# georgeretsi/smirk

Hardware: AMD Instinct MI355X
Metric: faces/sec (encode+FLAME+render+generate) @224x224 (higher is better)
Workload: dtype f32 results; encoder + generator convs as split-fp16 x3 MFMA with f32 accumulate (fp32-class error), FLAME / raster f32; 1 GPU; BASELINE config 4: full inference incl. SmirkGenerator re-synthesis, 1024-frame batch sharded over the GPUs; global_batch=1024, micro_batch=1024, image=224x224, parallelism=dp1, rccl_ranks_seen=1, collective=none (1 GPU), hw_queues=4

## Files before the change

### smirk_amd/csrc/conv_common.h

```cpp
#pragma once
#include "common.h"

#define CV_BK 32

typedef _Float16 half8 __attribute__((ext_vector_type(8)));

struct ConvArgs {
    SmirkConvDesc d;
    const float *in0, *in1, *w, *scale, *shift, *residual;
    float* out;
    int M, N, K, Cin;
    float* stats;
    int psh;
};

__device__ __forceinline__ void row_to_pixel(int m, int HoWo, int Wo, int psh, int& b, int& oy, int& ox) {
    b = m / HoWo;
    const int rem = m - b * HoWo;
    const int t = rem >> (2 * psh), in = rem & ((1 << (2 * psh)) - 1);
    const int tpr = Wo >> psh, ty = t / tpr, tx = t - ty * tpr;
    oy = (ty << psh) + (in >> psh);
    ox = (tx << psh) + (in & ((1 << psh) - 1));
}

// ... 66 lines not shown

static inline void conv_prof_next(const char* name, const ConvArgs& a) {
    if (!g_smirk_prof_on) return;
    const double px = (double)a.d.B * a.d.H * a.d.W;
    smirk_prof_next(name, 2.0 * a.M * a.N * a.K, 4.0 * (px * a.Cin + (double)a.M * a.N + (double)a.N * a.K + (a.residual ? (double)a.M * a.N : 0.0)));
}

bool smirk_conv3x3_ring64_eligible(const SmirkConvDesc* d, bool has_residual);
int smirk_conv3x3_ring64_launch(const SmirkConvDesc* d, const void* in0, const void* in1, const void* w, const float* scale, const float* shift, void* out,
                                void* pooled, hipStream_t st, float* stats = nullptr, int* stats_rows = nullptr);
bool smirk_conv3x3_upcat_eligible(int c, int H, int W);
size_t smirk_conv3x3_upcat_weff_bytes(int c);
size_t smirk_conv3x3_upcat_shift_bytes(int c);
int smirk_conv3x3_upcat_launch(int c, const void* d, const void* e, const SmirkConvLayer* up, const SmirkConvLayer* conv, void* out, int B, int H, int W,
                               void* weff, void* shift4, hipStream_t st);
bool smirk_conv3x3_patch_eligible(const SmirkConvDesc* d, bool has_residual);
int smirk_conv3x3_patch_launch(const SmirkConvDesc* d, const void* in0, const void* in1, const void* w, const float* scale,
                               const float* shift, void* out, hipStream_t st, const float* fw, const float* fb, float* fout,
                               int fcout);
#define HS_BM 256
#define HS_WGM 4
bool smirk_conv_halo_eligible(const ConvArgs& a);
int smirk_conv_halo_launch(const ConvArgs& a, hipStream_t st, bool x1);
bool smirk_conv_pp_eligible(const ConvArgs& a);
int smirk_conv_pp_launch(const ConvArgs& a, hipStream_t st);
```

### smirk_amd/csrc/conv_halo.hip

```cpp
#include <stdio.h>
#include <type_traits>

#include "conv_common.h"

#define HS_BN 128
#define HS_NSTAGE 3
#define HS_BRING_BYTES (HS_NSTAGE * HS_BN * 128)
#define HS_EPI_LD (2 * 32 + 4)
#define HS_DEFAULT_EB 0

typedef __attribute__((address_space(3))) void* hs_lptr_t;

template <int K>
using hs_ic = std::integral_constant<int, K>;

__device__ __forceinline__ int hs_b_off(int row, int stage, int piece) {
    return ((((row >> 3) * HS_NSTAGE + stage) << 8) + ((row & 7) << 5) + ((piece ^ ((row >> 1) & 7)) << 2)) * 4;
}

template <int NPA, int EB, bool X1, bool STATS = false>
__device__ __forceinline__ void conv_halo_body(const ConvArgs& a) {
    constexpr int NL = 3;
    extern __shared__ __attribute__((aligned(16))) float hs_smem[];
    char* lds = (char*)hs_smem;
    constexpr int ABUF = NPA * 8 * 1024;
    constexpr int ASTRIDE = ABUF + 128;
    constexpr int A0 = HS_BRING_BYTES;
    const SmirkConvDesc& d = a.d;
    const int tid = threadIdx.x, lane = tid & 63, wave = tid >> 6;
    const int swave = __builtin_amdgcn_readfirstlane(wave);
    const int wm = wave >> 1, wn = wave & 1;
    const int group = swave >> 2;
    const int ntn = a.N / HS_BN;
    const int logical = xcd_logical(blockIdx.x, gridDim.x);
    const int m0 = (logical / ntn) * HS_BM, n0 = (logical % ntn) * HS_BN;
    const int W = d.W, HW = d.H * d.W;
    const int fr = lane & 31, hb = lane >> 5;

    if (tid < 64) *(float*)(lds + A0 + (tid >> 5) * ASTRIDE + ABUF + (tid & 31) * 4) = 0.f;

    unsigned tabA[9];
    unsigned bB[2];
#pragma unroll
    for (int j = 0; j < 2; ++j) bB[j] = (unsigned)hs_b_off((wn * 2 + j) * 32 + fr, 0, 2 * hb);

    const int pos = lane & 7, lrow = lane >> 3;
    const unsigned colA16 = (unsigned)(pos ^ ((4 * (swave & 1) + (lrow >> 1)) & 7)) * 16u;
    const int qv0 = m0 - (W + 1) + 8 * swave + lrow;
    const int npix = d.B * HW;
    unsigned voffB[2];
#pragma unroll
    for (int p = 0; p < 2; ++p) {
        const int brow = 8 * (swave + 8 * p) + lrow;
        voffB[p] = ((unsigned)min(n0 + brow, a.N - 1) * (unsigned)a.K + (unsigned)(pos ^ ((brow >> 1) & 7)) * 4u) * 4u;
    }
    const __amdgpu_buffer_rsrc_t rs0 = __builtin_amdgcn_make_buffer_rsrc((void*)a.in0, (short)0, (int)((long long)npix * d.C0 * 4), 0x00020000);
    const __amdgpu_buffer_rsrc_t rs1 = __builtin_amdgcn_make_buffer_rsrc((void*)(d.C1 > 0 ? a.in1 : a.in0), (short)0,
                                                                         (int)((long long)npix * (d.C1 > 0 ? d.C1 : d.C0) * 4), 0x00020000);
    const __amdgpu_buffer_rsrc_t rsw = __builtin_amdgcn_make_buffer_rsrc((void*)a.w, (short)0, (int)((long long)a.N * a.K * 4), 0x00020000);
    const int sh0 = 31 - __builtin_clz((unsigned)d.C0) + 2, sh1 = d.C1 > 0 ? 31 - __builtin_clz((unsigned)d.C1) + 2 : sh0;
    const int ncc = (d.C0 + d.C1) / CV_BK;

    auto dmaA = [&](int cc, int abase, auto kc) {
        constexpr int KP = decltype(kc)::value;
        const int c0 = cc * CV_BK;
        const bool s1 = c0 >= d.C0;
        const int q = qv0 + 64 * KP;
        unsigned vo = ((unsigned)q << (s1 ? sh1 : sh0)) + colA16;
        vo = ((unsigned)q < (unsigned)npix) ? vo : 0x80000000u;
        const int so = (s1 ? c0 - d.C0 : c0) * 4;
        char* dst = lds + abase + (swave + 8 * KP) * 1024;
        if (s1) __builtin_amdgcn_raw_ptr_buffer_load_lds(rs1, (hs_lptr_t)dst, 16, vo, so, 0, 0);
        else __builtin_amdgcn_raw_ptr_buffer_load_lds(rs0, (hs_lptr_t)dst, 16, vo, so, 0, 0);
    };
    auto dmaB1 = [&](int cc, auto tapc, auto stc, auto pc) {
        constexpr int TAP = decltype(tapc)::value, ST = decltype(stc)::value, P = decltype(pc)::value;
        const int so = (TAP * a.Cin + cc * CV_BK) * 4;
        __builtin_amdgcn_raw_ptr_buffer_load_lds(rsw, (hs_lptr_t)(lds + (((swave + 8 * P) * HS_NSTAGE + ST) << 10)), 16, voffB[P], so, 0, 0);
    };
    auto dmaB = [&](int cc, auto tapc, auto stc) {
        dmaB1(cc, tapc, stc, hs_ic<0>{});
        dmaB1(cc, tapc, stc, hs_ic<1>{});
    };

    f32x16 acc0[2][2], acc1[2][2];
#pragma unroll
    for (int i = 0; i < 2; ++i)
#pragma unroll
        for (int j = 0; j < 2; ++j)
#pragma unroll
            for (int r = 0; r < 16; ++r) { acc0[i][j][r] = 0.f; acc1[i][j][r] = 0.f; }
    half8 ah[2][2], al[2][2], bh[2][2], bl[2][2];

    auto body = [&](int cc, int acur, int anext, auto tapc) {
        constexpr int TAP = decltype(tapc)::value, ST = TAP % 3;
        {
            const unsigned t = tabA[TAP];
            const unsigned a0 = (t & 0xffffu) + (unsigned)acur, a1 = (t >> 16) + (unsigned)acur;
            ah[0][0] = *(const half8*)(lds + a0);
            ah[1][0] = *(const half8*)(lds + (a0 ^ 64u));
            ah[0][1] = *(const half8*)(lds + a1);
            ah[1][1] = *(const half8*)(lds + (a1 ^ 64u));
            if constexpr (!X1) {
                al[0][0] = *(const half8*)(lds + (a0 ^ 16u)); al[1][0] = *(const half8*)(lds + (a0 ^ 80u));
                al[0][1] = *(const half8*)(lds + (a1 ^ 16u)); al[1][1] = *(const half8*)(lds + (a1 ^ 80u));
            }
#pragma unroll
            for (int j = 0; j < 2; ++j) {
                const unsigned b0 = bB[j];
                bh[0][j] = *(const half8*)(lds + b0 + ST * 1024);
                bh[1][j] = *(const half8*)(lds + (b0 ^ 64u) + ST * 1024);
                if constexpr (!X1) {
                    bl[0][j] = *(const half8*)(lds + (b0 ^ 16u) + ST * 1024);
                    bl[1][j] = *(const half8*)(lds + (b0 ^ 80u) + ST * 1024);
                }
            }
        }
        constexpr int T2 = (TAP + 2) % 9;
        constexpr int HASA = TAP < NPA ? 1 : 0, NDMA = 2 + HASA, NLD = NL < NDMA ? NL : NDMA;
        const int ccA = min(cc + 1, ncc - 1), ccB = min(cc + (TAP + 2 >= 9 ? 1 : 0), ncc - 1);
        auto dma = [&](auto kc) {
            constexpr int K = decltype(kc)::value;
            if constexpr (HASA && K == 0) dmaA(ccA, anext, hs_ic<(TAP < NPA ? TAP : 0)>{});
            else dmaB1(ccB, hs_ic<T2>{}, hs_ic<T2 % 3>{}, hs_ic<K - HASA>{});
        };
        if constexpr (NLD > 0) dma(hs_ic<0>{});
        if constexpr (NLD > 1) dma(hs_ic<1>{});
        if constexpr (NLD > 2) dma(hs_ic<2>{});
        if constexpr (NLD == 3) asm volatile("s_waitcnt vmcnt(3) lgkmcnt(0)" ::: "memory");
        else if constexpr (NLD == 2) asm volatile("s_waitcnt vmcnt(2) lgkmcnt(0)" ::: "memory");
        else if constexpr (NLD == 1) asm volatile("s_waitcnt vmcnt(1) lgkmcnt(0)" ::: "memory");
        else asm volatile("s_waitcnt vmcnt(0) lgkmcnt(0)" ::: "memory");
        __builtin_amdgcn_sched_barrier(0);
        __builtin_amdgcn_s_barrier();
        __builtin_amdgcn_sched_barrier(0);
        __builtin_amdgcn_s_setprio(1);
        auto mm_dma = [&](auto gc) {
            constexpr int G = decltype(gc)::value;
            if constexpr (NLD + G < NDMA) {
                __builtin_amdgcn_sched_barrier(0);
                dma(hs_ic<(NLD + G < NDMA ? NLD + G : 0)>{});
                __builtin_amdgcn_sched_barrier(0);
            }
        };
        auto mblock = [&](auto bc) {
            constexpr int BK = decltype(bc)::value;
#pragma unroll
            for (int j = 0; j < 2; ++j)
#pragma unroll
                for (int i = 0; i < 2; ++i) {
                    if constexpr (BK == 0) acc0[i][j] = __builtin_amdgcn_mfma_f32_32x32x16_f16(ah[0][i], bh[0][j], acc0[i][j], 0, 0, 0);
                    if constexpr (BK == 1 && !X1) acc1[i][j] = __builtin_amdgcn_mfma_f32_32x32x16_f16(ah[0][i], bl[0][j], acc1[i][j], 0, 0, 0);
// ... 10 lines not shown
        };
        mblock(hs_ic<0>{});
        mm_dma(hs_ic<0>{});
        mblock(hs_ic<1>{});
        mm_dma(hs_ic<1>{});
        mblock(hs_ic<2>{});
        mm_dma(hs_ic<2>{});
        mblock(hs_ic<3>{});
        if constexpr (EB == 8) hand_over();
        mblock(hs_ic<4>{});
        if constexpr (EB == 4) hand_over();
        mblock(hs_ic<5>{});
        __builtin_amdgcn_s_setprio(0);
        if constexpr (EB == 0) hand_over();
        else __builtin_amdgcn_sched_barrier(0);
    };

    dmaA(0, A0, hs_ic<0>{}); dmaA(0, A0, hs_ic<1>{}); dmaA(0, A0, hs_ic<2>{}); dmaA(0, A0, hs_ic<3>{}); dmaA(0, A0, hs_ic<4>{});
    if constexpr (NPA > 5) dmaA(0, A0, hs_ic<5>{});
    dmaB(0, hs_ic<0>{}, hs_ic<0>{});
    dmaB(0, hs_ic<1>{}, hs_ic<1>{});
    __builtin_amdgcn_sched_barrier(0);
    {
        unsigned ent[2][9];
#pragma unroll
        for (int i = 0; i < 2; ++i) {
            const int rl = (wm * 2 + i) * 32 + fr;
            const int m = m0 + rl;
            const int b = m / HW, rem = m - b * HW, y = rem / W, x = rem - y * W;
#pragma unroll
            for (int t = 0; t < 9; ++t) {
                int dy = t / 3 - 1, dx = t % 3 - 1;
                bool zero = m >= a.M;
                if (d.pad_mode == SMIRK_PAD_REFLECT) {
                    if (y + dy < 0 || y + dy >= d.H) dy = -dy;
                    if (x + dx < 0 || x + dx >= W) dx = -dx;
                } else {
                    zero = zero || y + dy < 0 || y + dy >= d.H || x + dx < 0 || x + dx >= W;
                }
                const int p = rl + (W + 1) + dy * W + dx;
                const unsigned off = (unsigned)p * 128u + (unsigned)(((2 * hb) ^ ((p >> 1) & 7)) << 4);
                ent[i][t] = zero ? (unsigned)ABUF : off;
            }
        }
#pragma unroll
        for (int t = 0; t < 9; ++t) tabA[t] = ent[0][t] | (ent[1][t] << 16);
    }
    asm volatile("s_waitcnt vmcnt(2) lgkmcnt(0)" ::: "memory");
    __builtin_amdgcn_s_barrier();
    __builtin_amdgcn_sched_barrier(0);
    if (group == 1) __builtin_amdgcn_s_barrier();
    for (int cc = 0; cc < ncc; ++cc) {
        const int acur = A0 + (cc & 1) * ASTRIDE, anext = A0 + ((cc + 1) & 1) * ASTRIDE;
        body(cc, acur, anext, hs_ic<0>{}); body(cc, acur, anext, hs_ic<1>{}); body(cc, acur, anext, hs_ic<2>{});
        body(cc, acur, anext, hs_ic<3>{}); body(cc, acur, anext, hs_ic<4>{}); body(cc, acur, anext, hs_ic<5>{});
        body(cc, acur, anext, hs_ic<6>{}); body(cc, acur, anext, hs_ic<7>{}); body(cc, acur, anext, hs_ic<8>{});
    }
    asm volatile("s_waitcnt vmcnt(0)" ::: "memory");
    float* ebuf = hs_smem + wave * 32 * HS_EPI_LD;
    constexpr int GPR = 8, ITEMS = 32 * GPR / 64;
    const int eg = lane & 7, erow = lane >> 3;
    const int en = n0 + wn * 64 + eg * 8;
    f32x4 sc0 = {1.f, 1.f, 1.f, 1.f}, sc1 = sc0, sf0 = {0.f, 0.f, 0.f, 0.f}, sf1 = sf0;
    if (a.scale) { sc0 = *(const f32x4*)(a.scale + en); sc1 = *(const f32x4*)(a.scale + en + 4); }
    if (a.shift) { sf0 = *(const f32x4*)(a.shift + en); sf1 = *(const f32x4*)(a.shift + en + 4); }
    half8 resh[2][ITEMS], resl[2][ITEMS];
    if (a.residual) {
#pragma unroll
        for (int i = 0; i < 2; ++i)
#pragma unroll
            for (int it = 0; it < ITEMS; ++it) {
                const int m = min(m0 + (wm * 2 + i) * 32 + it * 8 + erow, a.M - 1);
                const size_t o = (size_t)m * d.Cout + en;
                resh[i][it] = *(const half8*)(a.residual + o);
                resl[i][it] = *(const half8*)(a.residual + o + 4);
            }
    }
    __builtin_amdgcn_sched_barrier(0);
    if (group == 0) __builtin_amdgcn_s_barrier();
    __builtin_amdgcn_s_barrier();

    SmirkRangeAcc rng;
    float st1[2] = {0.f, 0.f}, st2[2] = {0.f, 0.f};
#pragma unroll
    for (int i = 0; i < 2; ++i) {
#pragma unroll
        for (int j = 0; j < 2; ++j) {
            float x16[16];
#pragma unroll
            for (int r = 0; r < 16; ++r) {
                x16[r] = X1 ? acc0[i][j][r] : acc0[i][j][r] + acc1[i][j][r] * (1.0f / 2048.0f);
                ebuf[mfma32_row(r, lane) * HS_EPI_LD + j * 32 + fr] = x16[r];
            }
            if constexpr (STATS) stats_block(x16, lane, a.M - (m0 + (wm * 2 + i) * 32), st1[j], st2[j]);
        }
        asm volatile("s_waitcnt lgkmcnt(0)" ::: "memory");
#pragma unroll
        for (int it = 0; it < ITEMS; ++it) {
            const int row = it * 8 + erow;
            const int m = m0 + (wm * 2 + i) * 32 + row;
            if (m < a.M) {
                float v[8];
                *(f32x4*)v = *(const f32x4*)(ebuf + row * HS_EPI_LD + eg * 8);
                *(f32x4*)(v + 4) = *(const f32x4*)(ebuf + row * HS_EPI_LD + eg * 8 + 4);
                const size_t o = (size_t)m * d.Cout + en;
                if (a.scale) {
#pragma unroll
                    for (int q = 0; q < 4; ++q) { v[q] *= sc0[q]; v[4 + q] *= sc1[q]; }
                }
                if (a.shift) {
#pragma unroll
                    for (int q = 0; q < 4; ++q) { v[q] += sf0[q]; v[4 + q] += sf1[q]; }
                }
                if (a.residual) {
#pragma unroll
                    for (int q = 0; q < 8; ++q) v[q] += join1(resh[i][it][q], resl[i][it][q]);
                }
                if (d.act == SMIRK_ACT_RELU) {
#pragma unroll
                    for (int q = 0; q < 8; ++q) v[q] = fmaxf(v[q], 0.f);
                }
                half8 hi, lo;
                split8(v, hi, lo, rng);
                *(half8*)(a.out + o) = hi;
                *(half8*)(a.out + o + 4) = lo;
            }
        }
        asm volatile("s_waitcnt lgkmcnt(0)" ::: "memory");
    }
    rng.commit();
    if constexpr (STATS) {
        float* prow = a.stats + (size_t)((m0 / HS_BM) * 4 + wm) * a.N * 2;
#pragma unroll
        for (int j = 0; j < 2; ++j) {
            const float t1 = stats_pair(st1[j]), t2 = stats_pair(st2[j]);
            const int n = n0 + wn * 64 + j * 32 + fr;
            if ((lane >> 5) == 0) { prow[n * 2] = t1; prow[n * 2 + 1] = t2; }
        }
    }
}

template <int NPA, int EB>
__global__ __launch_bounds__(512, 2) void conv_halo_kernel(ConvArgs a) { conv_halo_body<NPA, EB, false>(a); }
template <int NPA>
__global__ __launch_bounds__(512, 2) void conv_halo_x1_kernel(ConvArgs a) { conv_halo_body<NPA, 0, true>(a); }
template <int NPA, int EB>
__global__ __launch_bounds__(512, 2) void conv_halo_stats_kernel(ConvArgs a) { conv_halo_body<NPA, EB, false, true>(a); }
template <int NPA>
__global__ __launch_bounds__(512, 2) void conv_halo_x1_stats_kernel(ConvArgs a) { conv_halo_body<NPA, 0, true, true>(a); }

bool smirk_conv_halo_eligible(const ConvArgs& a) {
    const SmirkConvDesc& d = a.d;
    if (!smirk_switch(SMIRK_SW_IGEMM_HALO)) return false;
    if (d.KH != 3 || d.KW != 3 || d.stride != 1 || d.out_mode != SMIRK_OUT_NHWC || d.pad_t != 1 || d.pad_l != 1) return false;
    if (d.Ho != d.H || d.Wo != d.W || d.W > 63 || d.W < 2 || d.H < 2) return false;
    if (d.C0 % CV_BK || d.C1 % CV_BK || (d.C0 & (d.C0 - 1)) || (d.C1 & (d.C1 - 1))) return false;
    if (a.N % HS_BN || a.N < HS_BN) return false;
    if (!conv_operands_fit32(a)) return false;
    if (a.M < 4 * HS_BM) return false;
    return true;
}

template <int NPA, int EB, bool X1>
static int hs_launch(const ConvArgs& a, hipStream_t st, size_t lds) {
    const void* fn = X1 ? (const void*)conv_halo_x1_kernel<NPA> : (const void*)conv_halo_kernel<NPA, EB>;
    const void* fns = X1 ? (const void*)conv_halo_x1_stats_kernel<NPA> : (const void*)conv_halo_stats_kernel<NPA, EB>;
    if (const int rc = smirk_raise_dynamic_lds(a.stats ? fns : fn, 160 * 1024)) return rc;
    const int ntm = (a.M + HS_BM - 1) / HS_BM, ntn = a.N / HS_BN;
    if (g_smirk_prof_on) {
        char nm[64];
        if (X1) snprintf(nm, sizeof(nm), "conv_halo_x1_kernel<%d>[256x128,8w,halo,f16x1]", NPA);
        else snprintf(nm, sizeof(nm), "conv_halo_kernel<%d,%d>[256x128,8w,halo]", NPA, EB);
        conv_prof_next(nm, a);
    }
    if (a.stats) {
        if constexpr (X1) SMIRK_LAUNCH((conv_halo_x1_stats_kernel<NPA>), dim3(ntm * ntn), dim3(512), lds, st, a);
        else SMIRK_LAUNCH((conv_halo_stats_kernel<NPA, EB>), dim3(ntm * ntn), dim3(512), lds, st, a);
        return smirk_launch_status();
    }
    if constexpr (X1) SMIRK_LAUNCH((conv_halo_x1_kernel<NPA>), dim3(ntm * ntn), dim3(512), lds, st, a);
    else SMIRK_LAUNCH((conv_halo_kernel<NPA, EB>), dim3(ntm * ntn), dim3(512), lds, st, a);
    return smirk_launch_status();
}

int smirk_conv_halo_launch(const ConvArgs& a, hipStream_t st, bool x1) {
    const int npa = (HS_BM + 2 * (a.d.W + 1) + 63) / 64;
    const size_t lds = HS_BRING_BYTES + 2 * ((size_t)(npa <= 5 ? 5 : 6) * 8 * 1024 + 128);
    if (x1) return npa <= 5 ? hs_launch<5, HS_DEFAULT_EB, true>(a, st, lds) : hs_launch<6, HS_DEFAULT_EB, true>(a, st, lds);
    return npa <= 5 ? hs_launch<5, HS_DEFAULT_EB, false>(a, st, lds) : hs_launch<6, HS_DEFAULT_EB, false>(a, st, lds);
}
```

### smirk_amd/csrc/network.hip

```cpp
#include <sys/syscall.h>
#include <unistd.h>
#include <stdlib.h>

#include "conv_common.h"
#include "../../include/smirk_handoff.h"

namespace {

struct Arena {
    char* base;
    size_t off;
    void* take(size_t bytes) {
        off = smirk_align_up(off, 256);
        void* p = base ? base + off : nullptr;
        off += bytes;
        return p;
    }
};

struct Rot {
    void* slot[3];
    void* pick(const void* a, const void* b) const {
        for (int i = 0; i < 3; ++i)
            if (slot[i] != a && slot[i] != b) return slot[i];
        return nullptr;
    }
};

inline size_t act_bytes(int B, int H, int W, int C) { return (size_t)B * H * W * C * 4; }

struct GenPlan {
    void* x;
    void* e[4];
    Rot rot;
    void* upcat_w[2];
    void* upcat_s[2];
    size_t total;
};

GenPlan plan_generator(const SmirkGeneratorWeights* w, int B, int H, int W, void* ws) {
    Arena a{(char*)ws, 0};
    GenPlan p;
    const int f = w->features;
    p.x = a.take(act_bytes(B, H, W, w->cin_pad));
    for (int l = 0; l < 4; ++l) p.e[l] = a.take(act_bytes(B, H >> l, W >> l, f << l));
    const size_t big = act_bytes(B, H, W, f);
    for (int i = 0; i < 3; ++i) p.rot.slot[i] = a.take(big);
    for (int l = 0; l < 2; ++l) {
        const bool on = w->precision == SMIRK_PRECISION_F16X3 && f == 32;
        p.upcat_w[l] = on ? a.take(smirk_conv3x3_upcat_weff_bytes(f << l)) : nullptr;
        p.upcat_s[l] = on ? a.take(smirk_conv3x3_upcat_shift_bytes(f << l)) : nullptr;
    }
    p.total = smirk_align_up(a.off, 256);
    return p;
}

int conv_call(bool split, const SmirkConvDesc& d, const void* in0, const void* in1, const SmirkConvLayer& L, const void* residual, void* out,
              void* stream) {
    return split ? smirk_conv_igemm_f16x3(&d, in0, in1, L.w, L.scale, L.shift, residual, out, stream)
                 : smirk_conv_igemm_f32(&d, (const float*)in0, (const float*)in1, (const float*)L.w, L.scale, L.shift, (const float*)residual,
                                        (float*)out, stream);
}

SmirkConvDesc desc3x3(int B, int H, int W, int c0, int c1, int cout, bool reflect, bool relu) {
    SmirkConvDesc d;
    d.B = B; d.H = H; d.W = W; d.C0 = c0; d.C1 = c1; d.Cout = cout; d.KH = d.KW = 3; d.stride = 1; d.pad_t = d.pad_l = 1;
    d.Ho = H; d.Wo = W; d.pad_mode = reflect ? SMIRK_PAD_REFLECT : SMIRK_PAD_ZERO; d.act = relu ? SMIRK_ACT_RELU : SMIRK_ACT_NONE;
    d.out_mode = SMIRK_OUT_NHWC;
    return d;
}

SmirkConvDesc desc1x1(int B, int H, int W, int cin, int cout, bool relu, bool convt) {
    SmirkConvDesc d;
    d.B = B; d.H = H; d.W = W; d.C0 = cin; d.C1 = 0; d.Cout = cout; d.KH = d.KW = 1; d.stride = 1; d.pad_t = d.pad_l = 0;
    d.Ho = H; d.Wo = W; d.pad_mode = SMIRK_PAD_ZERO; d.act = relu ? SMIRK_ACT_RELU : SMIRK_ACT_NONE;
// ... 17 lines not shown
}

extern "C" size_t smirk_generator_workspace_bytes(const SmirkGeneratorWeights* w, int B, int H, int W) {
    if (!gen_args_ok(w, B, H, W)) return 0;
    return plan_generator(w, B, H, W, nullptr).total;
}

static int generator_forward_body(const SmirkGeneratorWeights* w, const float* a, int Ca, const float* b, int Cb, const void* packed, float* y, int B, int H,
                                  int W, void* const* taps, void* ws, size_t ws_bytes, void* stream) {
    const GenPlan p = plan_generator(w, B, H, W, ws);
    if (ws_bytes < p.total) return SMIRK_ERR_WORKSPACE;
    const bool split = w->precision == SMIRK_PRECISION_F16X3;
    const int f = w->features;

    if (packed) {
    } else if (split) {
        TRY(smirk_pack_generator_input_split16(a, Ca, b, Cb, p.x, B, H, W, stream));
    } else if (Cb == 0) {
        TRY(smirk_nchw_to_nhwc_pad(a, (float*)p.x, B, Ca, H, W, w->cin_pad, stream));
    } else {
        if (Ca != 3 || Cb != 3 || w->cin_pad != 8) return SMIRK_ERR_UNSUPPORTED;
        TRY(smirk_pack_generator_input(a, b, (float*)p.x, B, H, W, stream));
    }
    auto pool = [&](const void* in, void* out, int h, int wd, int c) {
        return split ? smirk_maxpool2x2_split16(in, out, B, h, wd, c, stream) : smirk_maxpool2x2_nhwc((const float*)in, (float*)out, B, h, wd, c, stream);
    };
    auto tap = [&](int i, const void* src, size_t bytes) {
        if (taps && taps[i]) (void)hipMemcpyAsync(taps[i], src, bytes, hipMemcpyDeviceToDevice, (hipStream_t)stream);
    };

    const int h16 = H >> 4, w16 = W >> 4, c16 = f << 4;
    const int L0 = 3;
    int nchain = 1;
    if (B >= 2 && !taps && !g_smirk_prof_on) {
        const double rounds = ((double)B * h16 * w16 / 256.0) * (c16 / 128.0) / smirk_device_cus();
        const double full = (double)(long long)(rounds + 0.999999);
        if (B >= 16 && full > 0 && (full - rounds) / full > 0.05) nchain = 2;
        if (const int forced = smirk_switch(SMIRK_SW_GEN_SPLIT_CHAINS)) nchain = forced;
        if (nchain > B) nchain = B;
    }
    hipStreamCaptureStatus cap = hipStreamCaptureStatusNone;
    if (nchain > 1 && (hipStreamIsCapturing((hipStream_t)stream, &cap) != hipSuccess || cap != hipStreamCaptureStatusNone)) { (void)hipGetLastError(); nchain = 1; }
    hipStream_t side[2] = {nullptr, nullptr};
    hipEvent_t fork = nullptr, join[2] = {nullptr, nullptr};
    if (nchain > 1) {
        struct ChainResources {
// ... 88 lines not shown
            void* pl = p.rot.pick(nullptr, nullptr);
            TRY(poolh(N(p.e[l], h, wd, c), Pw(pl), nb, h, wd, c, strm));
            cur = pl; cur_nat = false; ci = c;
        }
        const int c8 = f << 3;
        void* b1 = p.rot.pick(cur, nullptr);
        TRY(conv_call(split, desc3x3(nb, h16, w16, c8, 0, c16, false, true), P(cur), nullptr, w->enc[4][0], nullptr, Pw(b1), strm));
        void* b2 = p.rot.pick(b1, nullptr);
        TRY(conv_call(split, desc3x3(nb, h16, w16, c16, 0, c16, false, true), P(b1), nullptr, w->enc[4][1], nullptr, Pw(b2), strm));
        tap(4, b2, act_bytes(B, h16, w16, c16));
        const void* cur16 = b2;
        for (int k = 0; k < w->res_blocks; ++k) {
            void* t = p.rot.pick(cur16, nullptr);
            TRY(conv_call(split, desc3x3(nb, h16, w16, c16, 0, c16, true, true), P(cur16), nullptr, w->res[k][0], nullptr, Pw(t), strm));
            void* o = p.rot.pick(cur16, t);
            TRY(conv_call(split, desc3x3(nb, h16, w16, c16, 0, c16, true, false), P(t), nullptr, w->res[k][1], P(cur16), Pw(o), strm));
            cur16 = o;
        }
        tap(5, cur16, act_bytes(B, h16, w16, c16));
        const void* dc = cur16;
        for (int l = 3; l >= L0; --l) {
            const int h = H >> l, wd = W >> l, c = f << l;
            void* up = p.rot.pick(dc, nullptr);
            TRY(conv_call(split, desc1x1(nb, h / 2, wd / 2, 2 * c, c, false, true), P(dc), nullptr, w->up[3 - l], nullptr, Pw(up), strm));
            void* d1 = p.rot.pick(up, nullptr);
            TRY(conv_call(split, desc3x3(nb, h, wd, c, c, c, false, true), P(up), N(p.e[l], h, wd, c), w->dec[3 - l][0], nullptr, Pw(d1), strm));
            const bool last = l == L0;
            void* d2 = last ? p.rot.pick(d1, in) : p.rot.pick(d1, nullptr);
            TRY(conv_call(split, desc3x3(nb, h, wd, c, 0, c, false, true), P(d1), nullptr, w->dec[3 - l][1], nullptr, last ? Nw(d2, h, wd, c) : Pw(d2), strm));
            tap(6 + (3 - l), d2, act_bytes(B, h, wd, c));
            dc = d2;
        }
        out = dc;
        return SMIRK_OK;
    };
    const void* dcur = nullptr;
    if (nchain > 1) {
        int rc = hipEventRecord(fork, (hipStream_t)stream) == hipSuccess ? SMIRK_OK : SMIRK_ERR_LAUNCH;
        const void* last = nullptr;
        bool forked[2] = {false, false};
        for (int k = nchain - 1; rc == SMIRK_OK && k >= 0; --k) {
            const int b0 = (int)((long long)B * k / nchain), b1 = (int)((long long)B * (k + 1) / nchain);
            hipStream_t st_k = k == 0 ? (hipStream_t)stream : side[k - 1];
            if (k > 0 && hipStreamWaitEvent(st_k, fork, 0) != hipSuccess) { rc = SMIRK_ERR_LAUNCH; break; }
            if (k > 0) forked[k - 1] = true;
            rc = deep(k, b0, b1 - b0, (void*)st_k, cur, last);
            if (rc == SMIRK_OK && k > 0 && hipEventRecord(join[k - 1], st_k) != hipSuccess) rc = SMIRK_ERR_LAUNCH;
        }
        for (int k = 0; rc == SMIRK_OK && k + 1 < nchain; ++k)
            if (hipStreamWaitEvent((hipStream_t)stream, join[k], 0) != hipSuccess) rc = SMIRK_ERR_LAUNCH;
        if (rc != SMIRK_OK) {
            for (int k = 0; k < 2; ++k)
                if (forked[k]) (void)hipStreamSynchronize(side[k]);
            return rc;
        }
        dcur = last;
    } else {
        TRY(deep(0, 0, B, stream, cur, dcur));
    }
    for (int l = L0 - 1; l >= 0; --l) {
        const int h = H >> l, wd = W >> l, c = f << l;
        void* t1;
        if (l < 2 && split && f == 32 && smirk_conv3x3_upcat_eligible(c, h, wd)) {
            t1 = p.rot.pick(dcur, nullptr);
            TRY(smirk_conv3x3_upcat_launch(c, dcur, p.e[l], &w->up[3 - l], &w->dec[3 - l][0], t1, B, h, wd, p.upcat_w[l], p.upcat_s[l], (hipStream_t)stream));
        } else {
            void* up = p.rot.pick(dcur, nullptr);
            TRY(conv_call(split, desc1x1(B, h / 2, wd / 2, 2 * c, c, false, true), dcur, nullptr, w->up[3 - l], nullptr, up, stream));
            t1 = p.rot.pick(up, nullptr);
            TRY(conv_call(split, desc3x3(B, h, wd, c, c, c, false, true), up, p.e[l], w->dec[3 - l][0], nullptr, t1, stream));
        }
        if (l == 0 && split && !taps && f == 32 && H >= 64) {
            SmirkConvDesc d = desc3x3(B, h, wd, c, 0, c, false, true);
            const int rc = smirk_conv3x3_tail_f16x3(&d, t1, nullptr, w->dec[3][1].w, w->dec[3][1].scale, w->dec[3][1].shift, w->final_w, w->final_b,
                                                    y, w->out_channels, stream);
            if (rc != SMIRK_ERR_UNSUPPORTED) return rc;
        }
        void* t2 = p.rot.pick(t1, nullptr);
        TRY(conv_call(split, desc3x3(B, h, wd, c, 0, c, false, true), t1, nullptr, w->dec[3 - l][1], nullptr, t2, stream));
        tap(6 + (3 - l), t2, act_bytes(B, h, wd, c));
        dcur = t2;
    }
    return split ? smirk_conv1x1_sigmoid_nchw_split16(dcur, w->final_w, w->final_b, y, B, H, W, f, w->out_channels, stream)
                 : smirk_conv1x1_sigmoid_nchw((const float*)dcur, w->final_w, w->final_b, y, B, H, W, f, w->out_channels, stream);
}

extern "C" int smirk_generator_forward(const SmirkGeneratorWeights* w, const float* a, int Ca, const float* b, int Cb, float* y, int B, int H,
                                       int W, void* const* taps, void* ws, size_t ws_bytes, void* stream) {
// ... 164 lines not shown
```

Before: 11160 faces/sec.

## Compose deep-level upconv with decoder 3x3 into four-phase coarse conv

For the deep decoder levels (c=128,256), the 1x1 upsample conv and the first 3x3 decoder conv over its output are algebraically composed into four per-phase 2x2 convolutions on the coarse input. A compose kernel builds the combined weights and border-dependent shifts in double precision each call. The halo kernel gains an UP mode that writes the interleaved upsampled partial result, and the skip half is then added by a 3x3 conv with a residual. This removes the intermediate upsampled tensor round trip and the separate 1x1 pass. In exchange the MAC count on the coarse path rises and an extra compose launch is added.

```diff
diff --git a/smirk_amd/csrc/conv_common.h b/smirk_amd/csrc/conv_common.h
--- a/smirk_amd/csrc/conv_common.h
+++ b/smirk_amd/csrc/conv_common.h
@@ -112,5 +112,16 @@
 #define HS_WGM 4
 bool smirk_conv_halo_eligible(const ConvArgs& a);
 int smirk_conv_halo_launch(const ConvArgs& a, hipStream_t st, bool x1);
+struct SmirkUpdeepLevel {
+    int c;
+    const SmirkConvLayer *up, *conv;
+    void *weff, *shift16, *wskip;
+};
+size_t smirk_updeep_weff_bytes(int c);
+size_t smirk_updeep_shift_bytes(int c);
+size_t smirk_updeep_wskip_bytes(int c);
+bool smirk_updeep_eligible(int B, int H, int W, int c);
+int smirk_updeep_compose(const SmirkUpdeepLevel* lv, int nlv, hipStream_t st);
+int smirk_updeep_coarse_launch(const SmirkUpdeepLevel* lv, const void* d, void* partial, int B, int H, int W, hipStream_t st);
 bool smirk_conv_pp_eligible(const ConvArgs& a);
 int smirk_conv_pp_launch(const ConvArgs& a, hipStream_t st);
diff --git a/smirk_amd/csrc/conv_halo.hip b/smirk_amd/csrc/conv_halo.hip
--- a/smirk_amd/csrc/conv_halo.hip
+++ b/smirk_amd/csrc/conv_halo.hip
@@ -14,39 +14,45 @@
 template <int K>
 using hs_ic = std::integral_constant<int, K>;
 
+template <int NST = HS_NSTAGE>
 __device__ __forceinline__ int hs_b_off(int row, int stage, int piece) {
-    return ((((row >> 3) * HS_NSTAGE + stage) << 8) + ((row & 7) << 5) + ((piece ^ ((row >> 1) & 7)) << 2)) * 4;
-}
-
-template <int NPA, int EB, bool X1, bool STATS = false>
+    return ((((row >> 3) * NST + stage) << 8) + ((row & 7) << 5) + ((piece ^ ((row >> 1) & 7)) << 2)) * 4;
+}
+
+template <int NPA, int EB, bool X1, bool STATS = false, bool UP = false>
 __device__ __forceinline__ void conv_halo_body(const ConvArgs& a) {
-    constexpr int NL = 3;
+    constexpr int NTAP = UP ? 4 : 9, NST = UP ? 4 : HS_NSTAGE;
+    constexpr int NL = UP ? 4 : 3;
     extern __shared__ __attribute__((aligned(16))) float hs_smem[];
     char* lds = (char*)hs_smem;
     constexpr int ABUF = NPA * 8 * 1024;
     constexpr int ASTRIDE = ABUF + 128;
-    constexpr int A0 = HS_BRING_BYTES;
+    constexpr int A0 = NST * HS_BN * 128;
     const SmirkConvDesc& d = a.d;
     const int tid = threadIdx.x, lane = tid & 63, wave = tid >> 6;
     const int swave = __builtin_amdgcn_readfirstlane(wave);
     const int wm = wave >> 1, wn = wave & 1;
     const int group = swave >> 2;
     const int ntn = a.N / HS_BN;
-    const int logical = xcd_logical(blockIdx.x, gridDim.x);
+    int logical = xcd_logical(blockIdx.x, gridDim.x);
+    int cls = 0;
+    if constexpr (UP) { const int ntile = (int)gridDim.x >> 2; cls = logical / ntile; logical -= cls * ntile; }
+    const int dyc = cls >> 1, dxc = cls & 1;
     const int m0 = (logical / ntn) * HS_BM, n0 = (logical % ntn) * HS_BN;
     const int W = d.W, HW = d.H * d.W;
+    const float* const wcls = UP ? a.w + (size_t)cls * a.N * a.K : a.w;
     const int fr = lane & 31, hb = lane >> 5;
 
     if (tid < 64) *(float*)(lds + A0 + (tid >> 5) * ASTRIDE + ABUF + (tid & 31) * 4) = 0.f;
 
-    unsigned tabA[9];
+    unsigned tabA[NTAP];
     unsigned bB[2];
 #pragma unroll
-    for (int j = 0; j < 2; ++j) bB[j] = (unsigned)hs_b_off((wn * 2 + j) * 32 + fr, 0, 2 * hb);
+    for (int j = 0; j < 2; ++j) bB[j] = (unsigned)hs_b_off<NST>((wn * 2 + j) * 32 + fr, 0, 2 * hb);
 
     const int pos = lane & 7, lrow = lane >> 3;
     const unsigned colA16 = (unsigned)(pos ^ ((4 * (swave & 1) + (lrow >> 1)) & 7)) * 16u;
-    const int qv0 = m0 - (W + 1) + 8 * swave + lrow;
+    const int qv0 = m0 + (UP ? (dyc - 1) * W + (dxc - 1) : -(W + 1)) + 8 * swave + lrow;
     const int npix = d.B * HW;
     unsigned voffB[2];
 #pragma unroll
@@ -57,7 +63,7 @@
     const __amdgpu_buffer_rsrc_t rs0 = __builtin_amdgcn_make_buffer_rsrc((void*)a.in0, (short)0, (int)((long long)npix * d.C0 * 4), 0x00020000);
     const __amdgpu_buffer_rsrc_t rs1 = __builtin_amdgcn_make_buffer_rsrc((void*)(d.C1 > 0 ? a.in1 : a.in0), (short)0,
                                                                          (int)((long long)npix * (d.C1 > 0 ? d.C1 : d.C0) * 4), 0x00020000);
-    const __amdgpu_buffer_rsrc_t rsw = __builtin_amdgcn_make_buffer_rsrc((void*)a.w, (short)0, (int)((long long)a.N * a.K * 4), 0x00020000);
+    const __amdgpu_buffer_rsrc_t rsw = __builtin_amdgcn_make_buffer_rsrc((void*)wcls, (short)0, (int)((long long)a.N * a.K * 4), 0x00020000);
     const int sh0 = 31 - __builtin_clz((unsigned)d.C0) + 2, sh1 = d.C1 > 0 ? 31 - __builtin_clz((unsigned)d.C1) + 2 : sh0;
     const int ncc = (d.C0 + d.C1) / CV_BK;
 
@@ -76,7 +82,7 @@
     auto dmaB1 = [&](int cc, auto tapc, auto stc, auto pc) {
         constexpr int TAP = decltype(tapc)::value, ST = decltype(stc)::value, P = decltype(pc)::value;
         const int so = (TAP * a.Cin + cc * CV_BK) * 4;
-        __builtin_amdgcn_raw_ptr_buffer_load_lds(rsw, (hs_lptr_t)(lds + (((swave + 8 * P) * HS_NSTAGE + ST) << 10)), 16, voffB[P], so, 0, 0);
+        __builtin_amdgcn_raw_ptr_buffer_load_lds(rsw, (hs_lptr_t)(lds + (((swave + 8 * P) * NST + ST) << 10)), 16, voffB[P], so, 0, 0);
     };
     auto dmaB = [&](int cc, auto tapc, auto stc) {
         dmaB1(cc, tapc, stc, hs_ic<0>{});
@@ -93,7 +99,7 @@
     half8 ah[2][2], al[2][2], bh[2][2], bl[2][2];
 
     auto body = [&](int cc, int acur, int anext, auto tapc) {
-        constexpr int TAP = decltype(tapc)::value, ST = TAP % 3;
+        constexpr int TAP = decltype(tapc)::value, ST = TAP % NST;
         {
             const unsigned t = tabA[TAP];
             const unsigned a0 = (t & 0xffffu) + (unsigned)acur, a1 = (t >> 16) + (unsigned)acur;
@@ -116,18 +122,20 @@
                 }
             }
         }
-        constexpr int T2 = (TAP + 2) % 9;
-        constexpr int HASA = TAP < NPA ? 1 : 0, NDMA = 2 + HASA, NLD = NL < NDMA ? NL : NDMA;
-        const int ccA = min(cc + 1, ncc - 1), ccB = min(cc + (TAP + 2 >= 9 ? 1 : 0), ncc - 1);
+        constexpr int T2 = (TAP + 2) % NTAP;
+        constexpr int HASA = UP ? (TAP < 3 ? 1 + (TAP + 3 < NPA ? 1 : 0) : 0) : (TAP < NPA ? 1 : 0), NDMA = 2 + HASA, NLD = NL < NDMA ? NL : NDMA;
+        const int ccA = min(cc + 1, ncc - 1), ccB = min(cc + (TAP + 2 >= NTAP ? 1 : 0), ncc - 1);
         auto dma = [&](auto kc) {
             constexpr int K = decltype(kc)::value;
-            if constexpr (HASA && K == 0) dmaA(ccA, anext, hs_ic<(TAP < NPA ? TAP : 0)>{});
-            else dmaB1(ccB, hs_ic<T2>{}, hs_ic<T2 % 3>{}, hs_ic<K - HASA>{});
+            if constexpr (K < HASA) dmaA(ccA, anext, hs_ic<(TAP + 3 * K < NPA ? TAP + 3 * K : 0)>{});
+            else dmaB1(ccB, hs_ic<T2>{}, hs_ic<T2 % NST>{}, hs_ic<(K - HASA) & 1>{});
         };
         if constexpr (NLD > 0) dma(hs_ic<0>{});
         if constexpr (NLD > 1) dma(hs_ic<1>{});
         if constexpr (NLD > 2) dma(hs_ic<2>{});
-        if constexpr (NLD == 3) asm volatile("s_waitcnt vmcnt(3) lgkmcnt(0)" ::: "memory");
+        if constexpr (NLD > 3) dma(hs_ic<3>{});
+        if constexpr (NLD == 4) asm volatile("s_waitcnt vmcnt(4) lgkmcnt(0)" ::: "memory");
+        else if constexpr (NLD == 3) asm volatile("s_waitcnt vmcnt(3) lgkmcnt(0)" ::: "memory");
         else if constexpr (NLD == 2) asm volatile("s_waitcnt vmcnt(2) lgkmcnt(0)" ::: "memory");
         else if constexpr (NLD == 1) asm volatile("s_waitcnt vmcnt(1) lgkmcnt(0)" ::: "memory");
         else asm volatile("s_waitcnt vmcnt(0) lgkmcnt(0)" ::: "memory");
@@ -184,14 +192,21 @@
     dmaB(0, hs_ic<1>{}, hs_ic<1>{});
     __builtin_amdgcn_sched_barrier(0);
     {
-        unsigned ent[2][9];
+        unsigned ent[2][NTAP];
 #pragma unroll
         for (int i = 0; i < 2; ++i) {
             const int rl = (wm * 2 + i) * 32 + fr;
             const int m = m0 + rl;
             const int b = m / HW, rem = m - b * HW, y = rem / W, x = rem - y * W;
 #pragma unroll
-            for (int t = 0; t < 9; ++t) {
+            for (int t = 0; t < NTAP; ++t) {
+                if constexpr (UP) {
+                    const int ta = t >> 1, tb = t & 1, ay = y + dyc - 1 + ta, ax = x + dxc - 1 + tb;
+                    const bool zero = m >= a.M || ay < 0 || ay >= d.H || ax < 0 || ax >= W;
+                    const int p = rl + ta * W + tb;
+                    ent[i][t] = zero ? (unsigned)ABUF : (unsigned)p * 128u + (unsigned)(((2 * hb) ^ ((p >> 1) & 7)) << 4);
+                    continue;
+                }
                 int dy = t / 3 - 1, dx = t % 3 - 1;
                 bool zero = m >= a.M;
                 if (d.pad_mode == SMIRK_PAD_REFLECT) {
@@ -206,7 +221,7 @@
             }
         }
 #pragma unroll
-        for (int t = 0; t < 9; ++t) tabA[t] = ent[0][t] | (ent[1][t] << 16);
+        for (int t = 0; t < NTAP; ++t) tabA[t] = ent[0][t] | (ent[1][t] << 16);
     }
     asm volatile("s_waitcnt vmcnt(2) lgkmcnt(0)" ::: "memory");
     __builtin_amdgcn_s_barrier();
@@ -215,8 +230,11 @@
     for (int cc = 0; cc < ncc; ++cc) {
         const int acur = A0 + (cc & 1) * ASTRIDE, anext = A0 + ((cc + 1) & 1) * ASTRIDE;
         body(cc, acur, anext, hs_ic<0>{}); body(cc, acur, anext, hs_ic<1>{}); body(cc, acur, anext, hs_ic<2>{});
-        body(cc, acur, anext, hs_ic<3>{}); body(cc, acur, anext, hs_ic<4>{}); body(cc, acur, anext, hs_ic<5>{});
-        body(cc, acur, anext, hs_ic<6>{}); body(cc, acur, anext, hs_ic<7>{}); body(cc, acur, anext, hs_ic<8>{});
+        body(cc, acur, anext, hs_ic<3>{});
+        if constexpr (!UP) {
+            body(cc, acur, anext, hs_ic<4>{}); body(cc, acur, anext, hs_ic<5>{});
+            body(cc, acur, anext, hs_ic<6>{}); body(cc, acur, anext, hs_ic<7>{}); body(cc, acur, anext, hs_ic<8>{});
+        }
     }
     asm volatile("s_waitcnt vmcnt(0)" ::: "memory");
     float* ebuf = hs_smem + wave * 32 * HS_EPI_LD;
@@ -225,9 +243,25 @@
     const int en = n0 + wn * 64 + eg * 8;
     f32x4 sc0 = {1.f, 1.f, 1.f, 1.f}, sc1 = sc0, sf0 = {0.f, 0.f, 0.f, 0.f}, sf1 = sf0;
     if (a.scale) { sc0 = *(const f32x4*)(a.scale + en); sc1 = *(const f32x4*)(a.scale + en + 4); }
-    if (a.shift) { sf0 = *(const f32x4*)(a.shift + en); sf1 = *(const f32x4*)(a.shift + en + 4); }
+    if (!UP && a.shift) { sf0 = *(const f32x4*)(a.shift + en); sf1 = *(const f32x4*)(a.shift + en + 4); }
     half8 resh[2][ITEMS], resl[2][ITEMS];
-    if (a.residual) {
+    size_t uo[2][ITEMS];
+    f32x4 us0[2][ITEMS], us1[2][ITEMS];
+    if constexpr (UP) {
+#pragma unroll
+        for (int i = 0; i < 2; ++i)
+#pragma unroll
+            for (int it = 0; it < ITEMS; ++it) {
+                const int m = min(m0 + (wm * 2 + i) * 32 + it * 8 + erow, a.M - 1);
+                const int b = m / HW, rem = m - b * HW, y = rem / W, x = rem - y * W;
+                const int re = y == (dyc ? d.H - 1 : 0), ce = x == (dxc ? W - 1 : 0);
+                uo[i][it] = (((size_t)b * (2 * d.H) + (2 * y + dyc)) * (size_t)(2 * W) + (2 * x + dxc)) * d.Cout + en;
+                const float* const srow = a.shift + (size_t)((cls * 2 + re) * 2 + ce) * a.N + en;
+                us0[i][it] = *(const f32x4*)srow;
+                us1[i][it] = *(const f32x4*)(srow + 4);
+            }
+    }
+    if (!UP && a.residual) {
 #pragma unroll
         for (int i = 0; i < 2; ++i)
 #pragma unroll
@@ -265,20 +299,23 @@
                 float v[8];
                 *(f32x4*)v = *(const f32x4*)(ebuf + row * HS_EPI_LD + eg * 8);
                 *(f32x4*)(v + 4) = *(const f32x4*)(ebuf + row * HS_EPI_LD + eg * 8 + 4);
-                const size_t o = (size_t)m * d.Cout + en;
+                const size_t o = UP ? uo[i][it] : (size_t)m * d.Cout + en;
                 if (a.scale) {
 #pragma unroll
                     for (int q = 0; q < 4; ++q) { v[q] *= sc0[q]; v[4 + q] *= sc1[q]; }
                 }
-                if (a.shift) {
+                if constexpr (UP) {
+#pragma unroll
+                    for (int q = 0; q < 4; ++q) { v[q] += us0[i][it][q]; v[4 + q] += us1[i][it][q]; }
+                } else if (a.shift) {
 #pragma unroll
                     for (int q = 0; q < 4; ++q) { v[q] += sf0[q]; v[4 + q] += sf1[q]; }
                 }
-                if (a.residual) {
+                if (!UP && a.residual) {
 #pragma unroll
                     for (int q = 0; q < 8; ++q) v[q] += join1(resh[i][it][q], resl[i][it][q]);
                 }
-                if (d.act == SMIRK_ACT_RELU) {
+                if (!UP && d.act == SMIRK_ACT_RELU) {
 #pragma unroll
                     for (int q = 0; q < 8; ++q) v[q] = fmaxf(v[q], 0.f);
                 }
@@ -310,6 +347,8 @@
 __global__ __launch_bounds__(512, 2) void conv_halo_stats_kernel(ConvArgs a) { conv_halo_body<NPA, EB, false, true>(a); }
 template <int NPA>
 __global__ __launch_bounds__(512, 2) void conv_halo_x1_stats_kernel(ConvArgs a) { conv_halo_body<NPA, 0, true, true>(a); }
+template <int NPA>
+__global__ __launch_bounds__(512, 2) void conv_halo_up_kernel(ConvArgs a) { conv_halo_body<NPA, 0, false, false, true>(a); }
 
 bool smirk_conv_halo_eligible(const ConvArgs& a) {
     const SmirkConvDesc& d = a.d;
@@ -351,3 +390,181 @@
     if (x1) return npa <= 5 ? hs_launch<5, HS_DEFAULT_EB, true>(a, st, lds) : hs_launch<6, HS_DEFAULT_EB, true>(a, st, lds);
     return npa <= 5 ? hs_launch<5, HS_DEFAULT_EB, false>(a, st, lds) : hs_launch<6, HS_DEFAULT_EB, false>(a, st, lds);
 }
+
+struct UpdeepLevelArgs {
+    const float *wup, *bup, *w3, *scale;
+    float *weff, *shift16, *wskip;
+    int c, blk0, ngemm, nshift;
+};
+struct UpdeepComposeArgs {
+    UpdeepLevelArgs lv[2];
+};
+
+__device__ __forceinline__ double hs_dec64(const _Float16* row, int k) {
+    return (double)(float)row[(k >> 3) * 16 + (k & 7)] + (double)(float)row[(k >> 3) * 16 + 8 + (k & 7)] * (1.0 / 2048.0);
+}
+
+__global__ __launch_bounds__(256) void updeep_compose_kernel(UpdeepComposeArgs args) {
+    __shared__ __attribute__((aligned(16))) double As[16][64];
+    __shared__ __attribute__((aligned(16))) double Bs[16][64];
+    __shared__ double S[9];
+    const int li = (int)blockIdx.x >= args.lv[1].blk0 ? 1 : 0;
+    const UpdeepLevelArgs& L = args.lv[li];
+    const int C = L.c, CIN = 2 * C, tid = threadIdx.x;
+    int r = (int)blockIdx.x - L.blk0;
+    const _Float16* const w3h = (const _Float16*)L.w3;
+    const _Float16* const wuh = (const _Float16*)L.wup;
+    if (r < L.ngemm) {
+        const int nci = CIN / 64, nco = C / 64;
+        const int ci0 = (r % nci) * 64, co0 = ((r / nci) % nco) * 64, ct = r / (nci * nco);
+        const int cls = ct >> 2, tap = ct & 3, dy = cls >> 1, dx = cls & 1, ca = dy - 1 + (tap >> 1), cb = dx - 1 + (tap & 1);
+        const int tx = tid & 15, ty = tid >> 4;
+        double acc[4][4];
+#pragma unroll
+        for (int i = 0; i < 4; ++i)
+#pragma unroll
+            for (int j = 0; j < 4; ++j) acc[i][j] = 0.0;
+        for (int fy = -1; fy <= 1; ++fy) {
+            if (((dy + fy) >> 1) != ca) continue;
+            for (int fx = -1; fx <= 1; ++fx) {
+                if (((dx + fx) >> 1) != cb) continue;
+                const int sub = ((dy + fy) & 1) * 2 + ((dx + fx) & 1), t3 = (fy + 1) * 3 + (fx + 1);
+                for (int cu0 = 0; cu0 < C; cu0 += 16) {
+                    if (tid < 128) {
+                        const int row = tid >> 1, g = tid & 1;
+                        const _Float16* const src = w3h + ((size_t)((co0 + row) * 9 + t3) * CIN + cu0 + g * 8) * 2;
+                        const half8 hi = *(const half8*)src, lo = *(const half8*)(src + 8);
+#pragma unroll
+                        for (int q = 0; q < 8; ++q) As[g * 8 + q][row] = (double)(float)hi[q] + (double)(float)lo[q] * (1.0 / 2048.0);
+                    } else {
+                        const int t2 = tid - 128, krow = t2 >> 3, g = t2 & 7;
+                        const _Float16* const src = wuh + ((size_t)(sub * C + cu0 + krow) * CIN + ci0 + g * 8) * 2;
+                        const half8 hi = *(const half8*)src, lo = *(const half8*)(src + 8);
+#pragma unroll
+                        for (int q = 0; q < 8; ++q) Bs[krow][g * 8 + q] = (double)(float)hi[q] + (double)(float)lo[q] * (1.0 / 2048.0);
+                    }
+                    __syncthreads();
+#pragma unroll
+                    for (int k = 0; k < 16; ++k) {
+                        double av[4], bv[4];
+#pragma unroll
+                        for (int i = 0; i < 4; ++i) { av[i] = As[k][ty * 4 + i]; bv[i] = Bs[k][tx * 4 + i]; }
+#pragma unroll
+                        for (int i = 0; i < 4; ++i)
+#pragma unroll
+                            for (int j = 0; j < 4; ++j) acc[i][j] = fma(av[i], bv[j], acc[i][j]);
+                    }
+                    __syncthreads();
+                }
+            }
+        }
+        _Float16* const weh = (_Float16*)L.weff;
+#pragma unroll
+        for (int i = 0; i < 4; ++i) {
+            const int co = co0 + ty * 4 + i, k = tap * CIN + ci0 + tx * 4;
+            _Float16* const dst = weh + ((size_t)(cls * C + co) * 4 * CIN) * 2 + (k >> 3) * 16 + (k & 7);
+#pragma unroll
+            for (int j = 0; j < 4; ++j) {
+                const float v = (float)acc[i][j];
+                const _Float16 hi = (_Float16)v;
+                dst[j] = hi;
+                dst[8 + j] = (_Float16)((v - (float)hi) * 2048.0f);
+            }
+        }
+        return;
+    }
+    r -= L.ngemm;
+    if (r < L.nshift) {
+        const int co = r, lane = tid & 63, wave = tid >> 6;
+        for (int t = wave; t < 9; t += 4) {
+            const _Float16* const w3row = w3h + ((size_t)(co * 9 + t) * CIN) * 2;
+            double s = 0.0;
+            for (int cu = lane; cu < C; cu += 64) s += hs_dec64(w3row, cu) * (double)L.bup[cu];
+#pragma unroll
+            for (int o = 32; o >= 1; o >>= 1) s += __shfl_xor(s, o, 64);
+            if (lane == 0) S[t] = s;
+        }
+        __syncthreads();
+        if (tid < 16) {
+            const int ce = tid & 1, re = (tid >> 1) & 1, cls = tid >> 2, dy = cls >> 1, dx = cls & 1;
+            double acc = 0.0;
+            for (int fy = -1; fy <= 1; ++fy) {
+                if (re && fy == (dy ? 1 : -1)) continue;
+                for (int fx = -1; fx <= 1; ++fx) {
+                    if (ce && fx == (dx ? 1 : -1)) continue;
+                    acc += S[(fy + 1) * 3 + (fx + 1)];
+                }
+            }
+            L.shift16[tid * C + co] = (float)((double)L.scale[co] * acc);
+        }
+        return;
+    }
+    r -= L.nshift;
+    {
+        const int ppr = C / 4, idx = r * 256 + tid;
+        if (idx < 9 * C * ppr) {
+            const int row = idx / ppr, pc = idx - row * ppr;
+            *(f32x4*)(L.wskip + (size_t)row * C + pc * 4) = *(const f32x4*)(L.w3 + (size_t)row * CIN + C + pc * 4);
+        }
+    }
+}
+
+size_t smirk_updeep_weff_bytes(int c) { return (size_t)4 * c * 8 * c * 4; }
+size_t smirk_updeep_shift_bytes(int c) { return (size_t)16 * c * 4; }
+size_t smirk_updeep_wskip_bytes(int c) { return (size_t)9 * c * c * 4; }
+
+static ConvArgs updeep_args(int B, int H, int W, int c0, int cout, int taps) {
+    ConvArgs a = {};
+    SmirkConvDesc& d = a.d;
+    d.B = B; d.H = H; d.W = W; d.C0 = c0; d.C1 = 0; d.Cout = cout; d.KH = d.KW = 3; d.stride = 1; d.pad_t = d.pad_l = 1; d.Ho = H; d.Wo = W;
+    d.pad_mode = SMIRK_PAD_ZERO; d.act = SMIRK_ACT_NONE; d.out_mode = SMIRK_OUT_NHWC;
+    a.Cin = c0; a.K = taps * c0; a.N = cout; a.M = B * H * W;
+    return a;
+}
+
+bool smirk_updeep_eligible(int B, int H, int W, int c) {
+    if (B <= 0 || H < 4 || W < 4 || (H & 1) || (W & 1) || (long long)B * H * W > (1ll << 30)) return false;
+    if (!conv_fits32((long long)B * H * W * c)) return false;
+    return smirk_conv_halo_eligible(updeep_args(B, H / 2, W / 2, 2 * c, c, 4)) && smirk_conv_halo_eligible(updeep_args(B, H, W, c, c, 9));
+}
+
+int smirk_updeep_compose(const SmirkUpdeepLevel* lv, int nlv, hipStream_t st) {
+    if (nlv < 1 || nlv > 2) return SMIRK_ERR_BAD_ARG;
+    UpdeepComposeArgs args = {};
+    int blk = 0;
+    double mac = 0.0, bytes = 0.0;
+    for (int i = 0; i < 2; ++i) {
+        UpdeepLevelArgs& L = args.lv[i];
+        L.blk0 = blk;
+        if (i >= nlv) continue;
+        const SmirkUpdeepLevel& s = lv[i];
+        const int c = s.c;
+        if (c < 64 || c % 64 || !s.up || !s.conv || !s.up->w || !s.up->shift || s.up->scale || !s.conv->w || !s.conv->scale || !s.weff || !s.shift16 || !s.wskip)
+            return SMIRK_ERR_BAD_ARG;
+        L.wup = (const float*)s.up->w; L.bup = s.up->shift; L.w3 = (const float*)s.conv->w; L.scale = s.conv->scale;
+        L.weff = (float*)s.weff; L.shift16 = (float*)s.shift16; L.wskip = (float*)s.wskip;
+        L.c = c; L.ngemm = 16 * (c / 64) * (2 * c / 64); L.nshift = c;
+        blk += L.ngemm + L.nshift + (9 * c * (c / 4) + 255) / 256;
+        mac += 4.0 * 9 * c * c * 2 * c;
+        bytes += 4.0 * (4.0 * c * 2 * c + 18.0 * c * c + 32.0 * c * c + 9.0 * c * c);
+    }
+    if (g_smirk_prof_on) smirk_prof_next("updeep_compose_kernel", 2.0 * mac, bytes);
+    SMIRK_LAUNCH(updeep_compose_kernel, dim3(blk), dim3(256), 0, st, args);
+    return smirk_launch_status();
+}
+
+int smirk_updeep_coarse_launch(const SmirkUpdeepLevel* lv, const void* d, void* partial, int B, int H, int W, hipStream_t st) {
+    if (!lv || !d || !partial || !smirk_updeep_eligible(B, H, W, lv->c)) return SMIRK_ERR_UNSUPPORTED;
+    ConvArgs a = updeep_args(B, H / 2, W / 2, 2 * lv->c, lv->c, 4);
+    a.in0 = (const float*)d; a.w = (const float*)lv->weff; a.scale = lv->conv->scale; a.shift = (const float*)lv->shift16; a.out = (float*)partial;
+    constexpr size_t lds = 4 * HS_BN * 128 + 2 * (5 * 8 * 1024 + 128);
+    if (const int rc = smirk_raise_dynamic_lds((const void*)conv_halo_up_kernel<5>, 160 * 1024)) return rc;
+    const int ntm = (a.M + HS_BM - 1) / HS_BM, ntn = a.N / HS_BN;
+    if (g_smirk_prof_on) {
+        const double px = (double)a.M;
+        smirk_prof_next("conv_halo_up_kernel<5>[256x128,8w,halo,composed upconv]", 2.0 * (4.0 * a.M) * a.N * a.K,
+                        4.0 * (px * a.Cin + 4.0 * px * a.N + 4.0 * a.N * a.K));
+    }
+    SMIRK_LAUNCH((conv_halo_up_kernel<5>), dim3(4 * ntm * ntn), dim3(512), lds, st, a);
+    return smirk_launch_status();
+}
diff --git a/smirk_amd/csrc/network.hip b/smirk_amd/csrc/network.hip
--- a/smirk_amd/csrc/network.hip
+++ b/smirk_amd/csrc/network.hip
@@ -35,6 +35,9 @@
     Rot rot;
     void* upcat_w[2];
     void* upcat_s[2];
+    void* updeep_w[2];
+    void* updeep_s[2];
+    void* updeep_k[2];
     size_t total;
 };
 
@@ -51,6 +54,12 @@
         p.upcat_w[l] = on ? a.take(smirk_conv3x3_upcat_weff_bytes(f << l)) : nullptr;
         p.upcat_s[l] = on ? a.take(smirk_conv3x3_upcat_shift_bytes(f << l)) : nullptr;
     }
+    for (int l = 2; l < 4; ++l) {
+        const bool on = w->precision == SMIRK_PRECISION_F16X3 && f == 32;
+        p.updeep_w[l - 2] = on ? a.take(smirk_updeep_weff_bytes(f << l)) : nullptr;
+        p.updeep_s[l - 2] = on ? a.take(smirk_updeep_shift_bytes(f << l)) : nullptr;
+        p.updeep_k[l - 2] = on ? a.take(smirk_updeep_wskip_bytes(f << l)) : nullptr;
+    }
     p.total = smirk_align_up(a.off, 256);
     return p;
 }
@@ -114,6 +123,24 @@
         if (Ca != 3 || Cb != 3 || w->cin_pad != 8) return SMIRK_ERR_UNSUPPORTED;
         TRY(smirk_pack_generator_input(a, b, (float*)p.x, B, H, W, stream));
     }
+    SmirkUpdeepLevel ud[2];
+    bool ud_on[2] = {false, false};
+    {
+        SmirkUpdeepLevel todo[2];
+        int n = 0;
+        for (int l = 2; l < 4; ++l) {
+            ud[l - 2] = SmirkUpdeepLevel{f << l, &w->up[3 - l], &w->dec[3 - l][0], p.updeep_w[l - 2], p.updeep_s[l - 2], p.updeep_k[l - 2]};
+            ud_on[l - 2] = split && f == 32 && smirk_updeep_eligible(B, H >> l, W >> l, f << l);
+            if (ud_on[l - 2]) todo[n++] = ud[l - 2];
+        }
+        if (n) TRY(smirk_updeep_compose(todo, n, (hipStream_t)stream));
+    }
+    auto updeep = [&](int l, int nb, int h, int wd, const void* coarse, const void* skip, void* partial, void* out, void* strm) -> int {
+        const SmirkUpdeepLevel& u = ud[l - 2];
+        TRY(smirk_updeep_coarse_launch(&u, coarse, partial, nb, h, wd, (hipStream_t)strm));
+        const SmirkConvLayer half{u.wskip, u.conv->scale, u.conv->shift};
+        return conv_call(true, desc3x3(nb, h, wd, u.c, 0, u.c, false, true), skip, nullptr, half, partial, out, strm);
+    };
     auto pool = [&](const void* in, void* out, int h, int wd, int c) {
         return split ? smirk_maxpool2x2_split16(in, out, B, h, wd, c, stream) : smirk_maxpool2x2_nhwc((const float*)in, (float*)out, B, h, wd, c, stream);
     };
@@ -248,9 +275,13 @@
         for (int l = 3; l >= L0; --l) {
             const int h = H >> l, wd = W >> l, c = f << l;
             void* up = p.rot.pick(dc, nullptr);
-            TRY(conv_call(split, desc1x1(nb, h / 2, wd / 2, 2 * c, c, false, true), P(dc), nullptr, w->up[3 - l], nullptr, Pw(up), strm));
             void* d1 = p.rot.pick(up, nullptr);
-            TRY(conv_call(split, desc3x3(nb, h, wd, c, c, c, false, true), P(up), N(p.e[l], h, wd, c), w->dec[3 - l][0], nullptr, Pw(d1), strm));
+            if (ud_on[l - 2] && smirk_updeep_eligible(nb, h, wd, c)) {
+                TRY(updeep(l, nb, h, wd, P(dc), N(p.e[l], h, wd, c), Pw(up), Pw(d1), strm));
+            } else {
+                TRY(conv_call(split, desc1x1(nb, h / 2, wd / 2, 2 * c, c, false, true), P(dc), nullptr, w->up[3 - l], nullptr, Pw(up), strm));
+                TRY(conv_call(split, desc3x3(nb, h, wd, c, c, c, false, true), P(up), N(p.e[l], h, wd, c), w->dec[3 - l][0], nullptr, Pw(d1), strm));
+            }
             const bool last = l == L0;
             void* d2 = last ? p.rot.pick(d1, in) : p.rot.pick(d1, nullptr);
             TRY(conv_call(split, desc3x3(nb, h, wd, c, 0, c, false, true), P(d1), nullptr, w->dec[3 - l][1], nullptr, last ? Nw(d2, h, wd, c) : Pw(d2), strm));
@@ -290,6 +321,10 @@
         if (l < 2 && split && f == 32 && smirk_conv3x3_upcat_eligible(c, h, wd)) {
             t1 = p.rot.pick(dcur, nullptr);
             TRY(smirk_conv3x3_upcat_launch(c, dcur, p.e[l], &w->up[3 - l], &w->dec[3 - l][0], t1, B, h, wd, p.upcat_w[l], p.upcat_s[l], (hipStream_t)stream));
+        } else if (l >= 2 && ud_on[l - 2]) {
+            void* pp = p.rot.pick(dcur, nullptr);
+            t1 = p.rot.pick(pp, nullptr);
+            TRY(updeep(l, B, h, wd, dcur, p.e[l], pp, t1, stream));
         } else {
             void* up = p.rot.pick(dcur, nullptr);
             TRY(conv_call(split, desc1x1(B, h / 2, wd / 2, 2 * c, c, false, true), dcur, nullptr, w->up[3 - l], nullptr, up, stream));
```

Result: faster. 11310 faces/sec, median of 6 (+1.3%).
